# mahdi-slh/DeformContact

Hardware: AMD Instinct MI355X
Metric: M edges/sec fwd+bwd, everyday-deform batch=32 per GPU (encoder hot path) (higher is better)
Workload: dtype f32 (hops, storage, accumulate); wide dense blocks fp16x2-split operands (3 fp16 MFMA products, fp32 accumulate), narrow ones bf16x3-split (6 products); 1 GPU; everyday-deform synthetic, B=32 sample pairs per GPU: soft 32x(1024 v, 6132 e) + rigid 32x(762 v, 4560 e); TAGConv encoder 2 layers/branch, hidden 256, K=3 (configs[1]); edges_per_gpu_step=342144, global_batch=32, settle_steps=150, hipgraph=True, two_stream_branches=True, merged_branches=False, segmented_adjacency_build=True, parallelism=dp1

## Files before the change

### deformcontact_amd/_lib.py

```python
from __future__ import annotations

import ctypes
import os
from ctypes import POINTER, c_char_p, c_float, c_int, c_int32, c_int64, c_void_p

_HERE = os.path.dirname(os.path.abspath(__file__))
SO_PATH = os.path.join(_HERE, "libdeformcontact_hip.so")

_lib = None

_vp = c_void_p
_SIGNATURES = {
    "dc_version": (c_int, []),
    "dc_last_error": (c_char_p, []),
    "dc_stream_capture_id": (c_int64, [_vp]),
    "dc_csr_workspace_bytes": (c_int64, [c_int64, c_int64]),
    "dc_csr_build": (c_int, [_vp, c_int64, c_int64, c_int, c_int, _vp, _vp, _vp, _vp, _vp, _vp,
                             _vp, c_int64, _vp]),
    "dc_graph_workspace_bytes": (c_int64, [c_int64, c_int64]),
    "dc_graph_build": (c_int, [_vp, c_int64, c_int64, c_int, _vp, _vp, _vp, _vp, _vp, _vp, _vp, _vp,
                               _vp, _vp, c_int64, _vp]),
    "dc_graph_build_parts": (c_int, [POINTER(_vp), POINTER(c_int64), POINTER(c_int64), POINTER(c_int64), c_int,
                                     c_int64, c_int, _vp, _vp, _vp, _vp, _vp, _vp, _vp, _vp, _vp, _vp, c_int64,
                                     _vp]),
# ... 12 lines not shown
                                             _vp]),
    "dc_attn_flash_fwd": (c_int, [_vp, c_int64, _vp, _vp, _vp, _vp, _vp, c_int64, c_int64, c_int64, c_int64, _vp,
                                  c_int64, _vp, _vp]),
    "dc_hop_chain_max_nodes": (c_int64, []),
    "dc_hop_chain_lds_request": (c_int64, []),
    "dc_hop_chain_f32": (c_int, [_vp, _vp, _vp, _vp, c_int64, POINTER(c_int64), c_int, _vp, c_int64, c_int64, c_int64,
                                 c_int, c_int, c_int, _vp, c_int, _vp]),
    "dc_spmm_f32_bias_act": (c_int, [_vp, _vp, _vp, _vp, c_int64, _vp, c_int, _vp, c_int64, c_int64, c_int64, _vp]),
    "dc_colsum_workspace_bytes": (c_int64, [c_int64, c_int64, c_int]),
    "dc_mask_colsum_f32": (c_int, [_vp, c_int64, _vp, c_int64, _vp, c_int64, c_int64, c_int64, _vp, c_int64, _vp, c_int,
                                   _vp]),
    "dc_gat_alpha_fwd": (c_int, [_vp, c_int64, _vp, _vp, _vp, _vp, c_int64, c_int64, _vp]),
    "dc_gat_alpha_bwd": (c_int, [_vp, c_int64, _vp, _vp, _vp, _vp, _vp, c_int64, c_int64, c_int64, _vp, c_int64, _vp, _vp,
                                 c_int, _vp]),
    "dc_spmm_f32_pack": (c_int, [_vp, _vp, _vp, _vp, c_int64, _vp, c_int64, c_int64, c_int64, c_int64, c_int64, _vp]),
    "dc_spmm_f32_window": (c_int, [_vp, _vp, _vp, _vp, c_int64, _vp, c_int64, _vp, c_int64, c_int64,
                                   c_int64, c_int64, _vp]),
    "dc_spmm_f32_rowmax_window": (c_int, [_vp, _vp, _vp, _vp, c_int64, _vp, c_int64, _vp, c_int64, c_int64,
                                          c_int64, _vp, c_int, c_int64, _vp]),
    "dc_tag_grouped_weight_prep": (c_int, [POINTER(_vp), c_int, c_int, c_int64, c_int64, POINTER(_vp),
                                           POINTER(_vp), POINTER(_vp), POINTER(_vp), _vp]),
    "dc_tag_grouped_fwd_h2p": (c_int, [_vp, c_int64, c_int, POINTER(c_int64), POINTER(c_int64), c_int64,
                                       POINTER(_vp), POINTER(_vp), c_int, _vp, c_int64, c_int64, c_int64, _vp,
                                       POINTER(_vp), _vp]),
    "dc_tag_grouped_mask_grad": (c_int, [POINTER(_vp), POINTER(c_int64), c_int, POINTER(c_int64),
                                         POINTER(c_int64), c_int64, _vp, c_int64, _vp, c_int64, c_int64, _vp,
                                         _vp, _vp]),
    "dc_tag_grouped_bwd_dw_workspace_bytes": (c_int64, [POINTER(c_int64), c_int, c_int64, c_int64, c_int]),
    "dc_tag_grouped_bwd_dw_h2": (c_int, [_vp, c_int64, POINTER(_vp), POINTER(c_int64), c_int, c_int,
                                         POINTER(c_int64), POINTER(c_int64), c_int64, POINTER(_vp),
# ... 63 lines not shown
    "dc_tag_linear_fwd_h2p": (c_int, [_vp, c_int64, _vp, _vp, c_int, _vp, c_int64, c_int64, c_int64, c_int64,
                                      _vp, _vp, _vp, c_int64, _vp]),
    "dc_tag_linear_fwd_h2p_exp": (c_int, [_vp, c_int64, _vp, _vp, c_int64, c_int64, c_int64, c_int64, _vp, _vp, _vp,
                                          c_int64, _vp]),
    "dc_tag_weight_prep": (c_int, [POINTER(_vp), c_int, c_int64, c_int64, _vp, _vp, _vp, _vp, _vp]),
    "dc_tag_weight_prep_zero": (c_int, [POINTER(_vp), c_int, c_int64, c_int64, _vp, _vp, _vp, _vp, _vp, c_int64, _vp]),
    "dc_rowabsmax_f32": (c_int, [_vp, c_int64, c_int64, c_int64, _vp, _vp]),
    "dc_tag_weight_rowmax": (c_int, [POINTER(_vp), c_int, c_int64, c_int64, _vp, _vp]),
    "dc_spmm_f32_rowmax": (c_int, [_vp, _vp, _vp, _vp, c_int64, _vp, c_int64, _vp, c_int64, c_int64,
                                   c_int64, _vp, c_int, _vp]),
    "dc_tag_pack_input": (c_int, [_vp, c_int64, _vp, c_int64, c_int64, c_int64, c_int64, c_int64, _vp]),
    "dc_tag_pack_weights": (c_int, [POINTER(_vp), c_int, _vp, c_int64, c_int64, c_int64, _vp]),
    "dc_tag_linear_fwd_narrow_ok": (c_int, [c_int64, c_int, c_int64, c_int64]),
    "dc_tag_linear_fwd_narrow": (c_int, [_vp, c_int64, POINTER(_vp), c_int, c_int64, _vp, c_int, _vp, c_int64, c_int64,
                                         c_int64, c_int64, _vp]),
    "dc_attn_softmax_rows": (c_int, [_vp, c_int64, c_int64, c_int64, c_int64, _vp, _vp]),
    "dc_attn_exp_rows": (c_int, [_vp, c_int64, c_int64, c_int64, c_int64, _vp, _vp]),
    "dc_attn_ds_rows": (c_int, [_vp, _vp, c_int64, c_int64, c_int64, _vp, _vp, _vp]),
    "dc_adam_flat": (c_int, [_vp, _vp, _vp, _vp, c_int64, _vp, c_float, c_float, c_float, c_float,
                             c_int, _vp]),
    "dc_compose_perm": (c_int, [_vp, _vp, _vp, _vp, c_int64, _vp]),
    "dc_gat_edge_softmax_fwd": (c_int, [_vp, _vp, _vp, _vp, c_float, _vp, c_int64, _vp]),
    "dc_gat_edge_softmax_bwd": (c_int, [_vp, _vp, _vp, _vp, c_float, _vp, _vp, _vp, _vp, c_int64,
                                        _vp]),
    "dc_sddmm_f32": (c_int, [_vp, _vp, _vp, c_int64, _vp, c_int64, _vp, c_int64, c_int64, _vp]),
    "dc_segment_sum_f32": (c_int, [_vp, _vp, _vp, _vp, c_int64, _vp]),
    "dc_gather_f32": (c_int, [_vp, _vp, _vp, _vp, c_int64, _vp]),
    "dc_gat_alpha_heads_fwd": (c_int, [_vp, c_int64, _vp, _vp, _vp, _vp, c_int64, c_int64, c_int64, _vp]),
    "dc_gat_edge_softmax_heads_fwd": (c_int, [_vp, _vp, _vp, _vp, c_float, _vp, c_int64, c_int64, _vp]),
    "dc_spmm_f32_heads_bias_act": (c_int, [_vp, _vp, _vp, _vp, c_int64, _vp, c_int, c_int, _vp, c_int64, c_int64,
# ... 134 lines not shown
```

### deformcontact_amd/csrc/dc_dense_narrow.hip

```cpp
#include "dc_dense.h"

#ifndef DC_NARROW_ABL
#define DC_NARROW_ABL 0
#endif

namespace dc {

struct NarrowParams {
    const float *x;
    int64_t ld;
    const float *w[kMaxSeg];
    int nseg, fi;
    const float *bias;
    float *out;
    int64_t ldo, N;
    int relu, ntiles;
};

constexpr int kNarrowFo = 256;


template <int KS, int MB>
__global__ void __launch_bounds__(256)
k_fwd_narrow(NarrowParams p) {
    constexpr int TR = 32 * MB;
    constexpr int SROWA = KS * 96 + 16;
    constexpr int PPR = 4 * KS;
    constexpr int TP = TR * PPR, NV = (TP + 255) / 256;
    constexpr int KP = 16 * KS;
    constexpr int kOffStage = ((TR * SROWA + 1023) / 1024) * 1024;
    constexpr int kLdsTiles = kOffStage + TR * 1024, kLdsW = kNarrowFo * (KP + 4) * 4;
    __shared__ __attribute__((aligned(1024))) char lds[kLdsTiles > kLdsW ? kLdsTiles : kLdsW];
    char *const sA = lds;
    float *const so = reinterpret_cast<float *>(lds + kOffStage);
    const int wid = __builtin_amdgcn_readfirstlane((int)(threadIdx.x >> 6)), lane = threadIdx.x & 63;
    const int c = lane & 31, h = lane >> 5;

    f32x4 xv[NV];
    auto load_tile = [&](int t) {
        const int64_t row0 = (int64_t)t * TR;
#pragma unroll
        for (int j = 0; j < NV; ++j) {
            const int q = (int)threadIdx.x + 256 * j;
            if (TP % 256 != 0 && q >= TP) continue;
            const int r = q / PPR, c4 = q - r * PPR;
            int64_t row = row0 + r;
            row = row < p.N ? row : p.N - 1;
            if (DC_NARROW_ABL & 8) xv[j] = f32x4{(float)row, 1.f, 2.f, 3.f};
            else xv[j] = *reinterpret_cast<const f32x4 *>(p.x + row * p.ld + 4 * c4);
        }
    };
    int t = blockIdx.x;
    if (t < p.ntiles) load_tile(t);

    constexpr int WROW = KP + 4;
    {
        float *wi = reinterpret_cast<float *>(lds);
        const int width = p.nseg * p.fi, per4 = kNarrowFo * p.fi / 4;
        constexpr int MAXQ = 8;
        f32x4 wv[kMaxSeg][MAXQ];
#pragma unroll
        for (int s = 0; s < kMaxSeg; ++s)
#pragma unroll
            for (int j = 0; j < MAXQ; ++j) {
                const int q = (int)threadIdx.x + 256 * j;
                if (!(DC_NARROW_ABL & 2) && s < p.nseg && q < per4) wv[s][j] = *reinterpret_cast<const f32x4 *>(p.w[s] + 4 * q);
            }
#pragma unroll
        for (int s = 0; s < kMaxSeg; ++s)
#pragma unroll
// ... 3 lines not shown
                    int o = (4 * q) / p.fi, f = 4 * q - o * p.fi;
#pragma unroll
                    for (int i = 0; i < 4; ++i) {
                        wi[o * WROW + s * p.fi + f] = wv[s][j][i];
                        if (++f == p.fi) f = 0, ++o;
                    }
                }
            }
        const int padw = KP - width;
        for (int e = threadIdx.x; e < kNarrowFo * padw; e += 256) {
            const int o = e / padw, f = e - o * padw;
            wi[o * WROW + width + f] = 0.f;
        }
    }
    __syncthreads();
    bf16x8 fb[2][KS][3];
#pragma unroll
    for (int nb = 0; nb < 2; ++nb) {
        const float *wr = reinterpret_cast<const float *>(lds) + (64 * wid + 32 * nb + c) * WROW + 8 * h;
#pragma unroll
        for (int ks = 0; ks < KS; ++ks) {
            const f32x4 v0 = *reinterpret_cast<const f32x4 *>(wr + 16 * ks);
            const f32x4 v1 = *reinterpret_cast<const f32x4 *>(wr + 16 * ks + 4);
#pragma unroll
            for (int j = 0; j < 8; ++j) {
                __bf16 hi, mid, lo;
                split1(j < 4 ? v0[j] : v1[j - 4], hi, mid, lo);
                fb[nb][ks][0][j] = hi, fb[nb][ks][1][j] = mid, fb[nb][ks][2][j] = lo;
            }
        }
    }
    __syncthreads();
    float bcol[2];
#pragma unroll
    for (int nb = 0; nb < 2; ++nb) bcol[nb] = p.bias ? p.bias[64 * wid + 32 * nb + c] : 0.f;
    const bool relu = p.relu != 0;

    auto store_tile = [&]() {
#pragma unroll
        for (int j = 0; j < NV; ++j) {
            const int q = (int)threadIdx.x + 256 * j;
            if (TP % 256 != 0 && q >= TP) continue;
            const int r = q / PPR, c4 = q - r * PPR;
            bf16x4 hi, mid, lo;
#pragma unroll
            for (int i = 0; i < 4; ++i) {
                __bf16 a, b, d;
// ... 8 lines not shown
    };

    auto store_rows = [&](int64_t row0) {
#pragma unroll 4
        for (int r = wid; r < TR; r += 4) {
            const int64_t row = row0 + r;
            const f32x4 v = *reinterpret_cast<const f32x4 *>(so + r * 256 + 4 * lane);
            if (row < p.N && (!(DC_NARROW_ABL & 4) || v[0] == 12345.678f)) *reinterpret_cast<f32x4 *>(p.out + row * p.ldo + 4 * lane) = v;
        }
    };
    int64_t prev_row0 = -1;
    for (; t < p.ntiles; t += gridDim.x) {
        const int64_t row0 = (int64_t)t * TR;
        if (!(DC_NARROW_ABL & 8)) store_tile();
        if (prev_row0 >= 0) store_rows(prev_row0);
        if (t + (int)gridDim.x < p.ntiles) load_tile(t + gridDim.x);
        lds_barrier();
        f32x16 acc[MB][2];
#pragma unroll
        for (int mb = 0; mb < MB; ++mb)
#pragma unroll
            for (int nb = 0; nb < 2; ++nb)
#pragma unroll
                for (int i = 0; i < 16; ++i) acc[mb][nb][i] = 0.f;
        constexpr int HI = 0, MID = 1, LO = 2;
        constexpr int pa6[6] = {LO, HI, MID, MID, HI, HI}, pb6[6] = {HI, LO, MID, HI, MID, HI};
#pragma unroll
        for (int ks = 0; ks < KS; ++ks) {
            bf16x8 fa[MB][3];
#pragma unroll
            for (int mb = 0; mb < MB; ++mb)
#pragma unroll
                for (int pl = 0; pl < 3; ++pl)
                    fa[mb][pl] = *reinterpret_cast<const bf16x8 *>(sA + (mb * 32 + c) * SROWA + ks * 96 + pl * 32 + h * 16);
#pragma unroll
            for (int tt = 0; tt < 6; ++tt)
#pragma unroll
                for (int mb = 0; mb < MB; ++mb)
#pragma unroll
                    for (int nb = 0; nb < 2; ++nb)
                        if (!(DC_NARROW_ABL & 1))
                            acc[mb][nb] = __builtin_amdgcn_mfma_f32_32x32x16_bf16(fa[mb][pa6[tt]], fb[nb][ks][pb6[tt]], acc[mb][nb], 0, 0, 0);
                        else
                            acc[mb][nb][tt] += (float)fa[mb][pa6[tt]][0] * (float)fb[nb][ks][pb6[tt]][0];
        }
#pragma unroll
        for (int mb = 0; mb < MB; ++mb)
#pragma unroll
            for (int nb = 0; nb < 2; ++nb)
#pragma unroll
                for (int r = 0; r < 16; ++r) {
                    float v = acc[mb][nb][r] + bcol[nb];
                    if (relu) v = fmaxf(v, 0.f);
                    if (!(DC_NARROW_ABL & 16) || r == 0)
                        so[(mb * 32 + (r & 3) + 8 * (r >> 2) + 4 * h) * 256 + 64 * wid + 32 * nb + c] = v;
                }
        lds_barrier();
        prev_row0 = row0;
    }
    if (prev_row0 >= 0) store_rows(prev_row0);
}

template <int KS>
static void narrow_launch(const NarrowParams &p0, hipStream_t hs) {
    NarrowParams p = p0;
    p.ntiles = (int)((p.N + 31) / 32);
    const unsigned grid = (unsigned)(p.ntiles < 256 ? p.ntiles : 256);
    DC_LAUNCH((k_fwd_narrow<KS, 1>), dim3(grid), dim3(256), 0, hs, p);
}

}

using namespace dc;

extern "C" int dc_tag_linear_fwd_narrow_ok(int64_t fi, int nseg, int64_t wpad, int64_t Fo) {
// ... 5 lines not shown
                                        const float *bias, int relu, float *out, int64_t ldo, int64_t N, int64_t wpad,
                                        int64_t Fo, dc_stream_t stream) {
    DC_REQUIRE(dc_tag_linear_fwd_narrow_ok(fi, nseg, wpad, Fo),
               "dc_tag_linear_fwd_narrow: needs Fo = 256, a padded reduction of 96 / 112 / 128 >= nseg * fi (got Fo=%lld wpad=%lld "
               "nseg=%d fi=%lld)", (long long)Fo, (long long)wpad, nseg, (long long)fi);
    DC_REQUIRE(N >= 0, "dc_tag_linear_fwd_narrow: negative N");
    if (N == 0) return DC_OK;
    DC_REQUIRE(slab && ws && out && ld >= wpad && ldo >= Fo, "dc_tag_linear_fwd_narrow: null pointer / short leading dimension");
    DC_REQUIRE(ld % 4 == 0 && ldo % 4 == 0 && ((uintptr_t)slab & 15) == 0 && ((uintptr_t)out & 15) == 0,
               "dc_tag_linear_fwd_narrow: rows of the slab and of the output must be 16-byte aligned");
    DC_REQUIRE(N < ((int64_t)1 << 31) - 64, "dc_tag_linear_fwd_narrow: too many rows");
    NarrowParams p{};
    p.x = slab, p.ld = ld, p.nseg = nseg, p.fi = (int)fi, p.bias = bias, p.out = out, p.ldo = ldo, p.N = N, p.relu = relu;
    for (int s = 0; s < nseg; ++s) {
        DC_REQUIRE(ws[s], "dc_tag_linear_fwd_narrow: null weight segment %d", s);
        p.w[s] = ws[s];
    }
    hipStream_t hs = (hipStream_t)stream;
    switch (wpad) {
    case 96: narrow_launch<6>(p, hs); break;
    case 112: narrow_launch<7>(p, hs); break;
    default: narrow_launch<8>(p, hs); break;
    }
    return check_launch("dc_tag_linear_fwd_narrow");
}
```

### deformcontact_amd/csrc/dc_spmm.hip

```cpp
#include <stdlib.h>

#include "dc_common.h"

#pragma clang fp contract(off)

namespace dc {

template <int VEC> struct Vec;
template <> struct Vec<1> { using T = float; };
template <> struct Vec<4> { using T = float4; };

__device__ __forceinline__ float vzero(float) { return 0.0f; }
__device__ __forceinline__ float4 vzero(float4) { return make_float4(0.f, 0.f, 0.f, 0.f); }

__device__ __forceinline__ void vaxpy(float &acc, float w, float v) {
    const float m = w * v;
    acc = acc + m;
}
__device__ __forceinline__ void vaxpy(float4 &acc, float w, const float4 &v) {
    const float mx = w * v.x, my = w * v.y, mz = w * v.z, mw = w * v.w;
    acc.x = acc.x + mx;
    acc.y = acc.y + my;
    acc.z = acc.z + mz;
    acc.w = acc.w + mw;
// ... 102 lines not shown
        ww[3] = row_share_f<3>(my_w), ww[4] = row_share_f<4>(my_w), ww[5] = row_share_f<5>(my_w);
        ww[6] = row_share_f<6>(my_w), ww[7] = row_share_f<7>(my_w);
    } else {
        const bool mine = sub < 8 && p + sub < end;
        const int my_s = mine ? other[p + sub] : 0;
        const float my_w = mine ? (w ? w[p + sub] : 1.0f) : 0.0f;
#pragma unroll
        for (int j = 0; j < 8; ++j) {
            s[j] = __shfl(my_s, j, L);
            ww[j] = __shfl(my_w, j, L);
        }
    }
}

template <int VEC, int L, int U>
__global__ void __launch_bounds__(256)
k_spmm_sub(const int32_t *__restrict__ ptr, const int32_t *__restrict__ other,
           const float *__restrict__ w, const float *__restrict__ x, int64_t ldx,
           const float *addend, int64_t ldadd, float *y, int64_t ldy,
           int64_t N, int F, int src_off, float *self_dst = nullptr, int pad_beg = 0, int pad_end = 0) {
    using V = typename Vec<VEC>::T;
    constexpr int kRows = 256 / L;
    const unsigned lb = xcd_remap(blockIdx.x, gridDim.x);
    const int64_t row = (int64_t)lb * kRows + threadIdx.x / L;
    if (row >= N) return;
    const int sub = threadIdx.x % L;
    const int beg = ptr[row], end = ptr[row + 1];
    if (self_dst) {
        for (int c = sub; c < F; c += L) self_dst[row * ldy + c] = x[row * ldx + c];
        for (int c = pad_beg + sub; c < pad_end; c += L) self_dst[row * ldy + c] = 0.f;
    }

    for (int c0 = 0; c0 < F; c0 += L * VEC) {
        const int c = c0 + sub * VEC;
        const bool act = c < F;
        V acc = (addend && act) ? *reinterpret_cast<const V *>(addend + row * ldadd + c) : vzero(V{});
        for (int p = beg; p < end; p += U) {
            int s[U];
// ... 8 lines not shown
                    s[j] = ok ? other[p + j] : 0;
                    ww[j] = ok ? (w ? w[p + j] : 1.0f) : 0.0f;
                }
            }
#pragma unroll
            for (int j = 0; j < U; ++j) {
                const bool ok = act && p + j < end;
                v[j] = ok ? *reinterpret_cast<const V *>(x + (int64_t)(s[j] - src_off) * ldx + c) : vzero(V{});
            }
#pragma unroll
            for (int j = 0; j < U; ++j)
                if (p + j < end) vaxpy(acc, ww[j], v[j]);
        }
        if (act) *reinterpret_cast<V *>(y + row * ldy + c) = acc;
    }
}

template <int VEC, int L, int U>
static void launch_sub(const int32_t *ptr, const int32_t *other, const float *w, const float *x,
                       int64_t ldx, const float *addend, int64_t ldadd, float *y, int64_t ldy,
                       int64_t N, int F, int src_off, hipStream_t stream, float *self_dst = nullptr,
                       int pad_beg = 0, int pad_end = 0) {
    constexpr int kRows = 256 / L;
    const unsigned grid = (unsigned)((N + kRows - 1) / kRows);
    DC_LAUNCH((k_spmm_sub<VEC, L, U>), dim3(grid), dim3(256), 0, stream, ptr, other, w, x,
                       ldx, addend, ldadd, y, ldy, N, F, src_off, self_dst, pad_beg, pad_end);
}

static inline bool aligned16(const void *p) { return ((uintptr_t)p & 15) == 0; }

// ... 331 lines not shown
    if (N == 0) return DC_OK;
    DC_REQUIRE(ptr && x && slab && (other || true), "dc_spmm_f32_pack: null pointer");
    DC_REQUIRE(N < (int64_t)INT32_MAX / 8 && ldx >= F && width >= 2 * F && wpad >= width && lds >= wpad,
               "dc_spmm_f32_pack: needs ldx >= F, width >= 2 F (block 1 exists), wpad >= width, lds >= wpad");
    DC_REQUIRE((const void *)x != (const void *)slab, "dc_spmm_f32_pack: the slab must not alias x");
    float *y = slab + F;
    if (F > 16)
        launch_sub<1, 32, 8>(ptr, other, w, x, ldx, nullptr, 0, y, lds, N, (int)F, 0, stream, slab, (int)width, (int)wpad);
    else if (F > 8)
        launch_sub<1, 16, 8>(ptr, other, w, x, ldx, nullptr, 0, y, lds, N, (int)F, 0, stream, slab, (int)width, (int)wpad);
    else
        launch_sub<1, 8, 8>(ptr, other, w, x, ldx, nullptr, 0, y, lds, N, (int)F, 0, stream, slab, (int)width, (int)wpad);
    return check_launch("dc_spmm_f32_pack");
}

extern "C" int dc_spmm_f32_window(const int32_t *ptr, const int32_t *other, const float *w,
                                  const float *x, int64_t ldx, const float *addend, int64_t ldadd,
                                  float *y, int64_t ldy, int64_t N, int64_t F, int64_t row_offset,
                                  dc_stream_t stream) {
    DC_REQUIRE(row_offset >= 0 && row_offset < (int64_t)INT32_MAX, "dc_spmm_f32_window: bad row_offset");
    return spmm_f32_impl(ptr, other, w, x, ldx, addend, ldadd, y, ldy, N, F, (int)row_offset, stream);
}

extern "C" int dc_spmm_bf16(const int32_t *ptr, const int32_t *other, const float *w,
                            const uint16_t *x, int64_t ldx, const void *addend, int64_t ldadd,
                            void *y, int64_t ldy, int64_t N, int64_t F, int y_is_f32,
                            dc_stream_t stream_) {
    hipStream_t stream = (hipStream_t)stream_;
    DC_REQUIRE(N >= 0 && F >= 0, "dc_spmm_bf16: negative size N=%lld F=%lld", (long long)N,
               (long long)F);
// ... 58 lines not shown
```

### deformcontact_amd/ops.py

```python
from __future__ import annotations

import ctypes
import math
import os
from typing import List, Optional

import torch

from . import _lib
from .deferred import resolve
from .graph import GraphIndex, SortedAdjacency, _require_cuda, capture_id, current_stream_ptr, graph_index


def _rowmajor(t: torch.Tensor, what: str, dtypes=(torch.float32,)) -> int:
    if t.dim() != 2 or t.dtype not in dtypes:
        raise ValueError(f"{what}: expected a 2-D tensor of {dtypes}, got {tuple(t.shape)} {t.dtype}")
    if t.size(1) > 1 and t.stride(1) != 1:
        raise ValueError(f"{what}: innermost dimension must be contiguous")
    return t.stride(0) if t.size(0) > 1 else max(t.stride(0), t.size(1))


def _vp_array(ptrs):
    return (ctypes.c_void_p * len(ptrs))(*ptrs)

# ... 113 lines not shown
    return g if (ok and g.stride(1) == 1) else g.contiguous()


MAX_SEG = 4

DIRECT_PARAM_GRAD = True


DENSE_SPLIT_BF16 = os.environ.get("DC_DENSE_SPLIT", "1") != "0"

DENSE_PRODUCTS = 6


NARROW_FWD = os.environ.get("DC_NARROW_FWD", "1") != "0"

DENSE_F16X2 = os.environ.get("DC_DENSE_F16X2", "1") != "0"


HOP_CHAIN = os.environ.get("DC_HOP_CHAIN", "1") != "0"
_CHAIN_MAX_NODES = None


def hop_chain_eligible(g, adj: SortedAdjacency, slab: torch.Tensor, f: int, k: int) -> bool:
    global _CHAIN_MAX_NODES
    seg = getattr(g, "_layout", None)
    if not HOP_CHAIN or seg is None or k < 1 or f % 32 != 0 or adj.row_offset:
        return False
    if _CHAIN_MAX_NODES is None:
        _CHAIN_MAX_NODES = int(_lib.lib().dc_hop_chain_max_nodes())
    return (0 < g._seg_max_nodes <= _CHAIN_MAX_NODES and slab.dtype == torch.float32 and slab.dim() == 2
# ... 62 lines not shown
        return slab, rowmax
    return None


def _hop_cache_put(g, key, x, slab, rowmax, dev):
    cache = g.__dict__.setdefault("_hop_cache", {})
    if key not in cache:
        while len(cache) >= _HOP_CACHE_ENTRIES:
            cache.pop(next(iter(cache)))
    cache[key] = (slab, rowmax, capture_id(dev), x, x._version)


FUSED_PACK = os.environ.get("DC_FUSED_PACK", "1") != "0"


def _build_input_slab(g: GraphIndex, x: torch.Tensor, k: int, want_rowmax: bool, into=None):
    n, fi = x.shape
    concat, width, wpad = tag_slab_geometry(fi, k)
    dev = x.device
    slab = into[0] if into is not None else _alloc_slab(n, wpad, dev)
    xin = x if (x.dim() == 2 and x.stride(1) == 1) else x.contiguous()
    adj = g.fwd if (g is not None and k >= 1) else None
    if (FUSED_PACK and adj is not None and not want_rowmax and fi <= 32 and not adj.row_offset and g.normalize
            and adj.ptr.numel() == n + 1):
        _lib.check(_lib.lib().dc_spmm_f32_pack(adj.ptr.data_ptr(), adj.other.data_ptr(), adj.w.data_ptr(),
                                               xin.data_ptr(), xin.stride(0), slab.data_ptr(), slab.stride(0), n, fi,
                                               width, wpad, current_stream_ptr(dev)), "dc_spmm_f32_pack")
        for j in range(1, k):
            hop(adj, slab[:, j * fi:(j + 1) * fi], out=slab[:, (j + 1) * fi:(j + 2) * fi], weighted=True)
        return slab, None
    _lib.check(_lib.lib().dc_tag_pack_input(xin.data_ptr(), xin.stride(0), slab.data_ptr(), slab.stride(0), n,
                                            fi, width, wpad, current_stream_ptr(dev)),
               "dc_tag_pack_input")
    rowmax = None
    if want_rowmax:
        rowmax = into[1] if into is not None else torch.empty(n, dtype=torch.float32, device=dev)
    chained_hops(g, slab, fi, k, backward=False, rowmax=rowmax)
    return slab, rowmax


def _tag_uses_h2(fi: int, k: int, fo: Optional[int] = None) -> bool:
    concat, _, wpad = tag_slab_geometry(fi, k)
# ... 103 lines not shown
        return "fp32"
    if _tag_uses_h2(fi, k, None if six else fo):
        return "h2"
    if not tag_slab_geometry(fi, k)[0]:
        return "split"
    return "narrow" if (NARROW_FWD and DENSE_PRODUCTS == 6 and narrow_ok) else "concat"


def _dense_operands(slab: torch.Tensor, fi: int, k: int, concat: bool):
    ld = slab.stride(0)
    if concat:
        return [slab], [ld], slab.size(1), 1
    return [slab[:, j * fi:(j + 1) * fi] for j in range(k + 1)], [ld] * (k + 1), fi, k + 1


def _tag_slab(g, x: torch.Tensor, weights, h2: bool, need_x: bool):
    n, fi = x.shape
    k = len(weights) - 1
    dev = x.device
    wpad = tag_slab_geometry(fi, k)[2]
    slab = _as_slab_block0(x, n, fi, wpad)
    if slab is None and k == 0 and wpad == fi and x.is_contiguous() and x.data_ptr() % 16 == 0:
        slab = x
    rowmax = prepped = None
    if slab is None:
        key = None
        if HOP_CACHE and g is not None and k >= 1 and not need_x:
            key = _hop_cache_key(x, k, wpad, h2)
            hit = _hop_cache_get(g, key, x, dev)
            if hit is not None:
                slab, rowmax = hit
        if slab is None:
            slab, rowmax = _build_input_slab(g, x, k, h2)
            if key is not None:
                _hop_cache_put(g, key, x, slab, rowmax, dev)
    else:
        rowmax = torch.empty(n, dtype=torch.float32, device=dev) if h2 else None
        zeroed = False
        if h2 and g is not None and hop_chain_eligible(g, g.fwd, slab, fi, k):
            fo = weights[0].size(0)
            prepped = _h2_weight_prep(_lib.lib(), [w.contiguous() for w in weights], k, fo, fi,
                                      need_x and fo % 16 == 0, dev, current_stream_ptr(dev), zero=rowmax)
            zeroed = True
        chained_hops(g, slab, fi, k, backward=False, rowmax=rowmax, rowmax_zeroed=zeroed)
    if h2 and k == 0:
        rowmax = rowabsmax(slab)
    return slab, rowmax, prepped

# ... 143 lines not shown
            raise NotImplementedError(f"TAGConv K={k} > {MAX_SEG - 1} is not supported by the fused dense block")
        dev = x.device
        L = _lib.lib()
        st = current_stream_ptr(dev)
        six = next_geom is SIX_PRODUCTS
        if six:
            next_geom = None
        ctx.empty = n == 0
        if ctx.empty:
            ctx.fi, ctx.has_bias = fi, bias is not None
            ctx.save_for_backward(*weights)
            return _tag_out_buffer(next_geom, n, fo, dev)
        concat, width, wpad = tag_slab_geometry(fi, k)
        path = _dense_path(fi, k, fo, six, concat and bool(L.dc_tag_linear_fwd_narrow_ok(fi, k + 1, wpad, fo)))
        need_x = ctx.needs_input_grad[1]
        slab, rowmax, prepped = _tag_slab(g, x, weights, path == "h2", need_x)
        ws = [w.contiguous() for w in weights]
        if concat and path != "narrow":
            ws = [_pack_weights(ws, fo, fi, wpad, st)]
        out = _tag_out_buffer(next_geom, n, fo, dev)
        ldo = out.stride(0)
        b = bias.contiguous() if bias is not None else None
        wt = wt_rowmax = None
        if path == "h2":
            if prepped is None:
                prepped = _h2_weight_prep(L, ws, k, fo, fi, need_x and fo % 16 == 0, dev, st)
            wmax, wimg, wt, wt_rowmax = prepped
            rc = L.dc_tag_linear_fwd_h2p(slab.data_ptr(), slab.stride(0), wimg.data_ptr(), _ptr(b), int(relu),
                                         out.data_ptr(), ldo, n, width, fo, rowmax.data_ptr(), wmax.data_ptr(),
                                         None, 0, st)
        elif path == "narrow":
            rc = L.dc_tag_linear_fwd_narrow(slab.data_ptr(), slab.stride(0), _ptr_array(ws), k + 1, fi, _ptr(b),
                                            int(relu), out.data_ptr(), ldo, n, wpad, fo, st)
        else:
            xs, ldxs, fi_eff, nseg = _dense_operands(slab, fi, k, concat)
            args = (_ptr_array(xs), _i64_array(ldxs), _ptr_array(ws), nseg, _ptr(b), int(relu), out.data_ptr(), ldo,
                    n, fi_eff, fo)
            rc = L.dc_tag_linear_fwd(*args, st) if path == "fp32" else L.dc_tag_linear_fwd_split(*args, DENSE_PRODUCTS, st)
        _lib.check(rc, "dc_tag_linear_fwd")
        ctx.g, ctx.k, ctx.fi, ctx.fo, ctx.has_bias, ctx.relu, ctx.concat, ctx.path = \
            g, k, fi, fo, bias is not None, relu, concat, path
        ctx.params, ctx.bias_param = weights, bias
        ctx.save_for_backward(slab, out if relu else None, rowmax, wt, wt_rowmax, *ws)
        return out

# ... 2024 lines not shown
```

### include/deformcontact.h

```cpp
#ifndef DEFORMCONTACT_H
#define DEFORMCONTACT_H

#include <stdint.h>

#ifdef __cplusplus
extern "C" {
#endif

#define DC_OK 0
#define DC_EINVAL (-1)
#define DC_ELAUNCH (-2)
#define DC_EWORKSPACE (-3)

typedef void *dc_stream_t;

#define DC_MAX_PARTS 4
#define DC_MAX_GROUPS 4
#define DC_GROUP_ALIGN 256

int dc_version(void);
const char *dc_last_error(void);
int64_t dc_stream_capture_id(dc_stream_t stream);

int64_t dc_csr_workspace_bytes(int64_t E, int64_t N);
// ... 55 lines not shown

#define DC_NEIGHBORS_ND_CHUNK 32
int dc_neighbors_nd_fill(const float *x, int64_t ldx, int64_t nx, const int64_t *batch_x, const float *y, int64_t ldy,
                         int64_t ny, const int64_t *batch_y, int64_t f, int cap, int exclude_self, int32_t *nbr,
                         int32_t *counts, dc_stream_t stream);

int dc_hash_i64(const int64_t *v, int64_t n, uint64_t *out, dc_stream_t stream);

int dc_spmm_f32(const int32_t *ptr, const int32_t *other, const float *w, const float *x,
                int64_t ldx, const float *addend, int64_t ldadd, float *y, int64_t ldy,
                int64_t N, int64_t F, dc_stream_t stream);

int dc_spmm_f32_pack(const int32_t *ptr, const int32_t *other, const float *w, const float *x, int64_t ldx,
                     float *slab, int64_t lds, int64_t N, int64_t F, int64_t width, int64_t wpad,
                     dc_stream_t stream);

int dc_spmm_f32_window(const int32_t *ptr, const int32_t *other, const float *w, const float *x,
                       int64_t ldx, const float *addend, int64_t ldadd, float *y, int64_t ldy,
                       int64_t N, int64_t F, int64_t row_offset, dc_stream_t stream);
int dc_spmm_f32_rowmax_window(const int32_t *ptr, const int32_t *other, const float *w, const float *x,
                              int64_t ldx, const float *addend, int64_t ldadd, float *y, int64_t ldy,
                              int64_t N, int64_t F, float *rowmax, int mode, int64_t row_offset,
                              dc_stream_t stream);

int dc_spmm_bf16(const int32_t *ptr, const int32_t *other, const float *w, const uint16_t *x,
                 int64_t ldx, const void *addend, int64_t ldadd, void *y, int64_t ldy, int64_t N,
                 int64_t F, int y_is_f32, dc_stream_t stream);

int dc_spmm_f32_rowmax(const int32_t *ptr, const int32_t *other, const float *w, const float *x,
                       int64_t ldx, const float *addend, int64_t ldadd, float *y, int64_t ldy,
// ... 31 lines not shown
                      int nseg, const float *bias, int relu, float *out, int64_t ldo,
                      int64_t N, int64_t Fi, int64_t Fo, dc_stream_t stream);

int dc_tag_linear_bwd_dx(const float *g, int64_t ldg, const float *out_for_mask, int64_t ldo,
                         const float *const *ws, int nseg, float *const *gxs,
                         const int64_t *ldgxs, int64_t N, int64_t Fi, int64_t Fo,
                         dc_stream_t stream);

int dc_tag_linear_fwd_split(const float *const *xs, const int64_t *ldxs, const float *const *ws,
                            int nseg, const float *bias, int relu, float *out, int64_t ldo,
                            int64_t N, int64_t Fi, int64_t Fo, int products, dc_stream_t stream);
int dc_tag_linear_fwd_narrow_ok(int64_t fi, int nseg, int64_t wpad, int64_t Fo);
int dc_tag_linear_fwd_narrow(const float *slab, int64_t ld, const float *const *ws, int nseg, int64_t fi,
                             const float *bias, int relu, float *out, int64_t ldo, int64_t N, int64_t wpad,
                             int64_t Fo, dc_stream_t stream);
int64_t dc_tag_linear_bwd_dx_split_workspace_bytes(int64_t Fi, int64_t Fo, int nseg);
int dc_tag_linear_bwd_dx_split(const float *g, int64_t ldg, const float *out_for_mask,
                               int64_t ldo, const float *const *ws, int nseg, float *const *gxs,
                               const int64_t *ldgxs, void *workspace, int64_t workspace_bytes,
                               int64_t N, int64_t Fi, int64_t Fo, int products, dc_stream_t stream);

int64_t dc_tag_linear_bwd_dw_workspace_bytes(int64_t N, int64_t Fi, int64_t Fo, int nseg);
int dc_tag_linear_bwd_dw(const float *g, int64_t ldg, const float *out_for_mask, int64_t ldo,
                         const float *const *xs, const int64_t *ldxs, int nseg,
                         float *const *gws, int ngw, int64_t gw_cols, float *gbias,
                         int accumulate, void *partials, int64_t partials_bytes, int64_t N,
                         int64_t Fi, int64_t Fo, dc_stream_t stream);
int dc_tag_linear_bwd_dw_split(const float *g, int64_t ldg, const float *out_for_mask,
                               int64_t ldo, const float *const *xs, const int64_t *ldxs, int nseg,
                               float *const *gws, int ngw, int64_t gw_cols, float *gbias,
// ... 304 lines not shown
```

Measured before the change: 545.9 M edges/s.

## Prebuild narrow bf16x3 weight image inside pack kernel and read it in narrow fwd

Instead of having every block of the narrow TAG forward kernel load fp32 weights into LDS and split them into bf16 hi/mid/lo fragments, a precomputed fragment image is built once per forward. That build is fused as extra blocks into the SpMM pack kernel, so it costs no extra launch. The narrow kernel then reads per-lane fragments straight from global memory, which drops the weight-staging LDS and one barrier. It also adds launch_bounds occupancy variants (2 waves/CU for KS 6/7) and an option to defer the next-tile prefetch for KS>6. The risks are extra register pressure and the global image reads.

```diff
diff --git a/deformcontact_amd/_lib.py b/deformcontact_amd/_lib.py
--- a/deformcontact_amd/_lib.py
+++ b/deformcontact_amd/_lib.py
@@ -50,6 +50,8 @@
     "dc_gat_alpha_bwd": (c_int, [_vp, c_int64, _vp, _vp, _vp, _vp, _vp, c_int64, c_int64, c_int64, _vp, c_int64, _vp, _vp,
                                  c_int, _vp]),
     "dc_spmm_f32_pack": (c_int, [_vp, _vp, _vp, _vp, c_int64, _vp, c_int64, c_int64, c_int64, c_int64, c_int64, _vp]),
+    "dc_spmm_f32_pack_wprep": (c_int, [_vp, _vp, _vp, _vp, c_int64, _vp, c_int64, c_int64, c_int64, c_int64, c_int64,
+                                       POINTER(_vp), c_int, _vp, _vp]),
     "dc_spmm_f32_window": (c_int, [_vp, _vp, _vp, _vp, c_int64, _vp, c_int64, _vp, c_int64, c_int64,
                                    c_int64, c_int64, _vp]),
     "dc_spmm_f32_rowmax_window": (c_int, [_vp, _vp, _vp, _vp, c_int64, _vp, c_int64, _vp, c_int64, c_int64,
@@ -143,6 +145,8 @@
     "dc_tag_linear_fwd_narrow_ok": (c_int, [c_int64, c_int, c_int64, c_int64]),
     "dc_tag_linear_fwd_narrow": (c_int, [_vp, c_int64, POINTER(_vp), c_int, c_int64, _vp, c_int, _vp, c_int64, c_int64,
                                          c_int64, c_int64, _vp]),
+    "dc_tag_narrow_wimage": (c_int, [POINTER(_vp), c_int, c_int64, c_int64, _vp, _vp]),
+    "dc_tag_linear_fwd_narrow_img": (c_int, [_vp, c_int64, _vp, _vp, c_int, _vp, c_int64, c_int64, c_int64, c_int64, _vp]),
     "dc_attn_softmax_rows": (c_int, [_vp, c_int64, c_int64, c_int64, c_int64, _vp, _vp]),
     "dc_attn_exp_rows": (c_int, [_vp, c_int64, c_int64, c_int64, c_int64, _vp, _vp]),
     "dc_attn_ds_rows": (c_int, [_vp, _vp, c_int64, c_int64, c_int64, _vp, _vp, _vp]),
diff --git a/deformcontact_amd/csrc/dc_dense_narrow.hip b/deformcontact_amd/csrc/dc_dense_narrow.hip
--- a/deformcontact_amd/csrc/dc_dense_narrow.hip
+++ b/deformcontact_amd/csrc/dc_dense_narrow.hip
@@ -1,4 +1,5 @@
 #include "dc_dense.h"
+#include "dc_narrow_image.h"
 
 #ifndef DC_NARROW_ABL
 #define DC_NARROW_ABL 0
@@ -17,43 +18,13 @@
     int relu, ntiles;
 };
 
-constexpr int kNarrowFo = 256;
-
-
-template <int KS, int MB>
-__global__ void __launch_bounds__(256)
-k_fwd_narrow(NarrowParams p) {
-    constexpr int TR = 32 * MB;
-    constexpr int SROWA = KS * 96 + 16;
-    constexpr int PPR = 4 * KS;
-    constexpr int TP = TR * PPR, NV = (TP + 255) / 256;
+
+template <int KS>
+__device__ __forceinline__ void narrow_self_weights(const NarrowParams &p, char *lds, bf16x8 (&fb)[2][KS][3]) {
     constexpr int KP = 16 * KS;
-    constexpr int kOffStage = ((TR * SROWA + 1023) / 1024) * 1024;
-    constexpr int kLdsTiles = kOffStage + TR * 1024, kLdsW = kNarrowFo * (KP + 4) * 4;
-    __shared__ __attribute__((aligned(1024))) char lds[kLdsTiles > kLdsW ? kLdsTiles : kLdsW];
-    char *const sA = lds;
-    float *const so = reinterpret_cast<float *>(lds + kOffStage);
+    constexpr int WROW = KP + 4;
     const int wid = __builtin_amdgcn_readfirstlane((int)(threadIdx.x >> 6)), lane = threadIdx.x & 63;
     const int c = lane & 31, h = lane >> 5;
-
-    f32x4 xv[NV];
-    auto load_tile = [&](int t) {
-        const int64_t row0 = (int64_t)t * TR;
-#pragma unroll
-        for (int j = 0; j < NV; ++j) {
-            const int q = (int)threadIdx.x + 256 * j;
-            if (TP % 256 != 0 && q >= TP) continue;
-            const int r = q / PPR, c4 = q - r * PPR;
-            int64_t row = row0 + r;
-            row = row < p.N ? row : p.N - 1;
-            if (DC_NARROW_ABL & 8) xv[j] = f32x4{(float)row, 1.f, 2.f, 3.f};
-            else xv[j] = *reinterpret_cast<const f32x4 *>(p.x + row * p.ld + 4 * c4);
-        }
-    };
-    int t = blockIdx.x;
-    if (t < p.ntiles) load_tile(t);
-
-    constexpr int WROW = KP + 4;
     {
         float *wi = reinterpret_cast<float *>(lds);
         const int width = p.nseg * p.fi, per4 = kNarrowFo * p.fi / 4;
@@ -87,7 +58,6 @@
         }
     }
     __syncthreads();
-    bf16x8 fb[2][KS][3];
 #pragma unroll
     for (int nb = 0; nb < 2; ++nb) {
         const float *wr = reinterpret_cast<const float *>(lds) + (64 * wid + 32 * nb + c) * WROW + 8 * h;
@@ -104,6 +74,58 @@
         }
     }
     __syncthreads();
+}
+
+template <int KS, int MB, bool WIMG, bool LATE>
+__device__ __forceinline__ void narrow_block(const NarrowParams &p, const bf16x8 *__restrict__ img) {
+    constexpr int TR = 32 * MB;
+    constexpr int SROWA = KS * 96 + 16;
+    constexpr int PPR = 4 * KS;
+    constexpr int TP = TR * PPR, NV = (TP + 255) / 256;
+    constexpr int KP = 16 * KS;
+    constexpr int kOffStage = ((TR * SROWA + 1023) / 1024) * 1024;
+    constexpr int kLdsTiles = kOffStage + TR * 1024, kLdsW = kNarrowFo * (KP + 4) * 4;
+    __shared__ __attribute__((aligned(1024))) char lds[(WIMG || kLdsTiles > kLdsW) ? kLdsTiles : kLdsW];
+    char *const sA = lds;
+    float *const so = reinterpret_cast<float *>(lds + kOffStage);
+    const int wid = __builtin_amdgcn_readfirstlane((int)(threadIdx.x >> 6)), lane = threadIdx.x & 63;
+    const int c = lane & 31, h = lane >> 5;
+
+    f32x4 xv[NV];
+    auto load_tile = [&](int t) {
+        const int64_t row0 = (int64_t)t * TR;
+#pragma unroll
+        for (int j = 0; j < NV; ++j) {
+            const int q = (int)threadIdx.x + 256 * j;
+            if (TP % 256 != 0 && q >= TP) continue;
+            const int r = q / PPR, c4 = q - r * PPR;
+            int64_t row = row0 + r;
+            row = row < p.N ? row : p.N - 1;
+            if (DC_NARROW_ABL & 8) xv[j] = f32x4{(float)row, 1.f, 2.f, 3.f};
+            else xv[j] = *reinterpret_cast<const f32x4 *>(p.x + row * p.ld + 4 * c4);
+        }
+    };
+    int t = blockIdx.x;
+    if (t < p.ntiles) load_tile(t);
+
+    bf16x8 fb[2][KS][3];
+    if constexpr (WIMG) {
+#pragma unroll
+        for (int ks = 0; ks < KS; ++ks)
+#pragma unroll
+            for (int pl = 0; pl < 3; ++pl)
+#pragma unroll
+                for (int nb = 0; nb < 2; ++nb) {
+                    if (DC_NARROW_ABL & 2) {
+#pragma unroll
+                        for (int j = 0; j < 8; ++j) fb[nb][ks][pl][j] = (__bf16)(float)(lane + ks + pl + nb);
+                    } else {
+                        fb[nb][ks][pl] = img[((ks * 3 + pl) * 8 + 2 * wid + nb) * 64 + lane];
+                    }
+                }
+    } else {
+        narrow_self_weights<KS>(p, lds, fb);
+    }
     float bcol[2];
 #pragma unroll
     for (int nb = 0; nb < 2; ++nb) bcol[nb] = p.bias ? p.bias[64 * wid + 32 * nb + c] : 0.f;
@@ -142,7 +164,7 @@
         const int64_t row0 = (int64_t)t * TR;
         if (!(DC_NARROW_ABL & 8)) store_tile();
         if (prev_row0 >= 0) store_rows(prev_row0);
-        if (t + (int)gridDim.x < p.ntiles) load_tile(t + gridDim.x);
+        if (!LATE && t + (int)gridDim.x < p.ntiles) load_tile(t + gridDim.x);
         lds_barrier();
         f32x16 acc[MB][2];
 #pragma unroll
@@ -172,6 +194,7 @@
                         else
                             acc[mb][nb][tt] += (float)fa[mb][pa6[tt]][0] * (float)fb[nb][ks][pb6[tt]][0];
         }
+        if (LATE && t + (int)gridDim.x < p.ntiles) load_tile(t + gridDim.x);
 #pragma unroll
         for (int mb = 0; mb < MB; ++mb)
 #pragma unroll
@@ -187,6 +210,30 @@
         prev_row0 = row0;
     }
     if (prev_row0 >= 0) store_rows(prev_row0);
+}
+
+template <int KS, int MB>
+__global__ void __launch_bounds__(256) k_fwd_narrow(NarrowParams p) { narrow_block<KS, MB, false, false>(p, nullptr); }
+
+template <int KS, int WPC>
+__global__ void __launch_bounds__(256, WPC) k_fwd_narrow_img(NarrowParams p, const bf16x8 *__restrict__ img) {
+    narrow_block<KS, 1, true, (WPC == 2 && KS > 6)>(p, img);
+}
+
+__global__ void __launch_bounds__(256) k_narrow_wimage(NarrowImageParams q) { narrow_image_fill(q, (int)blockIdx.x); }
+
+static int narrow_wpc() {
+    static const int v = env_int("DC_NARROW_WPC", 2) == 1 ? 1 : 2;
+    return v;
+}
+
+template <int KS, int WPC>
+static void narrow_img_launch(const NarrowParams &p0, const void *img, hipStream_t hs) {
+    NarrowParams p = p0;
+    p.ntiles = (int)((p.N + 31) / 32);
+    const int cap = 256 * (WPC == 2 ? narrow_wpc() : 1);
+    const unsigned grid = (unsigned)(p.ntiles < cap ? p.ntiles : cap);
+    DC_LAUNCH((k_fwd_narrow_img<KS, WPC>), dim3(grid), dim3(256), 0, hs, p, static_cast<const bf16x8 *>(img));
 }
 
 template <int KS>
@@ -222,6 +269,7 @@
     p.x = slab, p.ld = ld, p.nseg = nseg, p.fi = (int)fi, p.bias = bias, p.out = out, p.ldo = ldo, p.N = N, p.relu = relu;
     for (int s = 0; s < nseg; ++s) {
         DC_REQUIRE(ws[s], "dc_tag_linear_fwd_narrow: null weight segment %d", s);
+        DC_REQUIRE(al16(ws[s]), "dc_tag_linear_fwd_narrow: weight segment %d is not 16-byte aligned", s);
         p.w[s] = ws[s];
     }
     hipStream_t hs = (hipStream_t)stream;
@@ -232,3 +280,37 @@
     }
     return check_launch("dc_tag_linear_fwd_narrow");
 }
+
+extern "C" int dc_tag_narrow_wimage(const float *const *ws, int nseg, int64_t fi, int64_t wpad, void *wimg,
+                                    dc_stream_t stream) {
+    DC_REQUIRE(narrow_image_args_ok(ws, nseg, fi, wpad, wimg),
+               "dc_tag_narrow_wimage: needs 1..%d 4-byte-aligned weight segments [256, fi <= 32], a padded reduction of 96 / "
+               "112 / 128 >= nseg * fi and a 16-byte-aligned image (got nseg=%d fi=%lld wpad=%lld)", kMaxSeg, nseg,
+               (long long)fi, (long long)wpad);
+    const NarrowImageParams q = narrow_image_params(ws, nseg, fi, wpad, wimg);
+    DC_LAUNCH(k_narrow_wimage, dim3((unsigned)narrow_image_blocks(q.ks)), dim3(256), 0, (hipStream_t)stream, q);
+    return check_launch("dc_tag_narrow_wimage");
+}
+
+extern "C" int dc_tag_linear_fwd_narrow_img(const float *slab, int64_t ld, const void *wimg, const float *bias, int relu,
+                                            float *out, int64_t ldo, int64_t N, int64_t wpad, int64_t Fo,
+                                            dc_stream_t stream) {
+    DC_REQUIRE(Fo == kNarrowFo && (wpad == 96 || wpad == 112 || wpad == 128),
+               "dc_tag_linear_fwd_narrow_img: needs Fo = 256 and a padded reduction of 96 / 112 / 128 (got Fo=%lld wpad=%lld)",
+               (long long)Fo, (long long)wpad);
+    DC_REQUIRE(N >= 0, "dc_tag_linear_fwd_narrow_img: negative N");
+    if (N == 0) return DC_OK;
+    DC_REQUIRE(slab && wimg && out && ld >= wpad && ldo >= Fo, "dc_tag_linear_fwd_narrow_img: null pointer / short leading dimension");
+    DC_REQUIRE(ld % 4 == 0 && ldo % 4 == 0 && al16(slab) && al16(out) && al16(wimg),
+               "dc_tag_linear_fwd_narrow_img: rows of the slab and of the output and the image must be 16-byte aligned");
+    DC_REQUIRE(N < ((int64_t)1 << 31) - 64, "dc_tag_linear_fwd_narrow_img: too many rows");
+    NarrowParams p{};
+    p.x = slab, p.ld = ld, p.bias = bias, p.out = out, p.ldo = ldo, p.N = N, p.relu = relu;
+    hipStream_t hs = (hipStream_t)stream;
+    switch (wpad) {
+    case 96: narrow_img_launch<6, 2>(p, wimg, hs); break;
+    case 112: narrow_img_launch<7, 2>(p, wimg, hs); break;
+    default: narrow_img_launch<8, 1>(p, wimg, hs); break;
+    }
+    return check_launch("dc_tag_linear_fwd_narrow_img");
+}
diff --git a/deformcontact_amd/csrc/dc_narrow_image.h b/deformcontact_amd/csrc/dc_narrow_image.h
--- /dev/null
+++ b/deformcontact_amd/csrc/dc_narrow_image.h
@@ -0,0 +1,66 @@
+#pragma once
+#include "dc_dense.h"
+
+namespace dc {
+
+constexpr int kNarrowFo = 256;
+constexpr int kNarrowImgStepBytes = 3 * 8 * 64 * 16;
+
+struct NarrowImageParams {
+    const float *w[kMaxSeg];
+    int nseg, fi, ks;
+    void *img;
+};
+
+__host__ __device__ constexpr int narrow_image_items(int ks) { return kNarrowFo * 2 * ks; }
+__host__ __device__ constexpr int narrow_image_blocks(int ks) { return narrow_image_items(ks) / 256; }
+
+__device__ __forceinline__ void narrow_image_fill(const NarrowImageParams &p, int blk) {
+    const int id = blk * 256 + (int)threadIdx.x;
+    const int per = 2 * p.ks;
+    const int o = id / per, kh = id - o * per;
+    if (o >= kNarrowFo) return;
+    const int width = p.nseg * p.fi;
+    float v[8];
+    int s = (8 * kh) / p.fi, f = 8 * kh - s * p.fi;
+#pragma unroll
+    for (int j = 0; j < 8; ++j) {
+        v[j] = 0.f;
+        if (8 * kh + j < width) {
+            const float *ws = p.w[0];
+#pragma unroll
+            for (int q = 1; q < kMaxSeg; ++q) ws = s == q ? p.w[q] : ws;
+            v[j] = ws[o * p.fi + f];
+        }
+        if (++f == p.fi) f = 0, ++s;
+    }
+    bf16x8 pl[3];
+#pragma unroll
+    for (int j = 0; j < 8; ++j) {
+        __bf16 hi, mid, lo;
+        split1(v[j], hi, mid, lo);
+        pl[0][j] = hi, pl[1][j] = mid, pl[2][j] = lo;
+    }
+    const int ks = kh >> 1, h = kh & 1, lane = (o & 31) + 32 * h;
+    char *dst = static_cast<char *>(p.img) + (size_t)ks * kNarrowImgStepBytes + ((o >> 5) * 64 + lane) * 16;
+#pragma unroll
+    for (int q = 0; q < 3; ++q) *reinterpret_cast<bf16x8 *>(dst + q * (8 * 64 * 16)) = pl[q];
+}
+
+inline bool narrow_image_args_ok(const float *const *ws, int nseg, int64_t fi, int64_t wpad, const void *img) {
+    if (!ws || !img || nseg < 1 || nseg > kMaxSeg || fi < 1 || fi > 32 || nseg * fi > wpad) return false;
+    if (wpad != 96 && wpad != 112 && wpad != 128) return false;
+    if ((uintptr_t)img & 15) return false;
+    for (int s = 0; s < nseg; ++s)
+        if (!ws[s] || ((uintptr_t)ws[s] & 3)) return false;
+    return true;
+}
+
+inline NarrowImageParams narrow_image_params(const float *const *ws, int nseg, int64_t fi, int64_t wpad, void *img) {
+    NarrowImageParams q{};
+    for (int s = 0; s < nseg; ++s) q.w[s] = ws[s];
+    q.nseg = nseg, q.fi = (int)fi, q.ks = (int)(wpad / 16), q.img = img;
+    return q;
+}
+
+}
diff --git a/deformcontact_amd/csrc/dc_spmm.hip b/deformcontact_amd/csrc/dc_spmm.hip
--- a/deformcontact_amd/csrc/dc_spmm.hip
+++ b/deformcontact_amd/csrc/dc_spmm.hip
@@ -1,6 +1,7 @@
 #include <stdlib.h>
 
 #include "dc_common.h"
+#include "dc_narrow_image.h"
 
 #pragma clang fp contract(off)
 
@@ -140,14 +141,13 @@
 }
 
 template <int VEC, int L, int U>
-__global__ void __launch_bounds__(256)
-k_spmm_sub(const int32_t *__restrict__ ptr, const int32_t *__restrict__ other,
-           const float *__restrict__ w, const float *__restrict__ x, int64_t ldx,
-           const float *addend, int64_t ldadd, float *y, int64_t ldy,
-           int64_t N, int F, int src_off, float *self_dst = nullptr, int pad_beg = 0, int pad_end = 0) {
+__device__ __forceinline__ void
+spmm_sub_rows(unsigned lb, const int32_t *__restrict__ ptr, const int32_t *__restrict__ other,
+              const float *__restrict__ w, const float *__restrict__ x, int64_t ldx,
+              const float *addend, int64_t ldadd, float *y, int64_t ldy,
+              int64_t N, int F, int src_off, float *self_dst, int pad_beg, int pad_end) {
     using V = typename Vec<VEC>::T;
     constexpr int kRows = 256 / L;
-    const unsigned lb = xcd_remap(blockIdx.x, gridDim.x);
     const int64_t row = (int64_t)lb * kRows + threadIdx.x / L;
     if (row >= N) return;
     const int sub = threadIdx.x % L;
@@ -186,6 +186,30 @@
         }
         if (act) *reinterpret_cast<V *>(y + row * ldy + c) = acc;
     }
+}
+
+template <int VEC, int L, int U>
+__global__ void __launch_bounds__(256)
+k_spmm_sub(const int32_t *__restrict__ ptr, const int32_t *__restrict__ other,
+           const float *__restrict__ w, const float *__restrict__ x, int64_t ldx,
+           const float *addend, int64_t ldadd, float *y, int64_t ldy,
+           int64_t N, int F, int src_off, float *self_dst = nullptr, int pad_beg = 0, int pad_end = 0) {
+    spmm_sub_rows<VEC, L, U>(xcd_remap(blockIdx.x, gridDim.x), ptr, other, w, x, ldx, addend, ldadd, y, ldy, N, F, src_off,
+                             self_dst, pad_beg, pad_end);
+}
+
+template <int L, int U>
+__global__ void __launch_bounds__(256)
+k_spmm_sub_wimg(const int32_t *__restrict__ ptr, const int32_t *__restrict__ other,
+                const float *__restrict__ w, const float *__restrict__ x, int64_t ldx, float *y, int64_t ldy,
+                int64_t N, int F, float *self_dst, int pad_beg, int pad_end, NarrowImageParams img) {
+    const unsigned nimg = (unsigned)narrow_image_blocks(img.ks);
+    if (blockIdx.x < nimg) {
+        narrow_image_fill(img, (int)blockIdx.x);
+        return;
+    }
+    spmm_sub_rows<1, L, U>(xcd_remap(blockIdx.x - nimg, gridDim.x - nimg), ptr, other, w, x, ldx, nullptr, 0, y, ldy, N, F, 0,
+                           self_dst, pad_beg, pad_end);
 }
 
 template <int VEC, int L, int U>
@@ -547,6 +571,40 @@
     return check_launch("dc_spmm_f32_pack");
 }
 
+template <int L>
+static void launch_pack_wimg(const int32_t *ptr, const int32_t *other, const float *w, const float *x, int64_t ldx,
+                             float *slab, int64_t lds, int64_t N, int F, int width, int wpad,
+                             const NarrowImageParams &img, hipStream_t stream) {
+    constexpr int kRows = 256 / L;
+    const unsigned grid = (unsigned)((N + kRows - 1) / kRows) + (unsigned)narrow_image_blocks(img.ks);
+    DC_LAUNCH((k_spmm_sub_wimg<L, 8>), dim3(grid), dim3(256), 0, stream, ptr, other, w, x, ldx, slab + F, lds, N, F, slab,
+              width, wpad, img);
+}
+
+extern "C" int dc_spmm_f32_pack_wprep(const int32_t *ptr, const int32_t *other, const float *w, const float *x,
+                                      int64_t ldx, float *slab, int64_t lds, int64_t N, int64_t F, int64_t width,
+                                      int64_t wpad, const float *const *ws, int nseg, void *wimg, dc_stream_t stream_) {
+    hipStream_t stream = (hipStream_t)stream_;
+    DC_REQUIRE(N >= 1 && F >= 1 && F <= 32, "dc_spmm_f32_pack_wprep: at least one row of 1..32 floats (got N=%lld F=%lld)",
+               (long long)N, (long long)F);
+    DC_REQUIRE(ptr && x && slab, "dc_spmm_f32_pack_wprep: null pointer");
+    DC_REQUIRE(N < (int64_t)INT32_MAX / 8 && ldx >= F && width >= 2 * F && wpad >= width && lds >= wpad,
+               "dc_spmm_f32_pack_wprep: needs ldx >= F, width >= 2 F (block 1 exists), wpad >= width, lds >= wpad");
+    DC_REQUIRE((const void *)x != (const void *)slab, "dc_spmm_f32_pack_wprep: the slab must not alias x");
+    DC_REQUIRE(width == (int64_t)nseg * F && narrow_image_args_ok(ws, nseg, F, wpad, wimg),
+               "dc_spmm_f32_pack_wprep: needs 1..%d 4-byte-aligned weight segments with nseg * F = width, a padded width of "
+               "96 / 112 / 128 and a 16-byte-aligned image (got nseg=%d F=%lld width=%lld wpad=%lld)", kMaxSeg, nseg,
+               (long long)F, (long long)width, (long long)wpad);
+    const NarrowImageParams img = narrow_image_params(ws, nseg, F, wpad, wimg);
+    if (F > 16)
+        launch_pack_wimg<32>(ptr, other, w, x, ldx, slab, lds, N, (int)F, (int)width, (int)wpad, img, stream);
+    else if (F > 8)
+        launch_pack_wimg<16>(ptr, other, w, x, ldx, slab, lds, N, (int)F, (int)width, (int)wpad, img, stream);
+    else
+        launch_pack_wimg<8>(ptr, other, w, x, ldx, slab, lds, N, (int)F, (int)width, (int)wpad, img, stream);
+    return check_launch("dc_spmm_f32_pack_wprep");
+}
+
 extern "C" int dc_spmm_f32_window(const int32_t *ptr, const int32_t *other, const float *w,
                                   const float *x, int64_t ldx, const float *addend, int64_t ldadd,
                                   float *y, int64_t ldy, int64_t N, int64_t F, int64_t row_offset,
diff --git a/deformcontact_amd/ops.py b/deformcontact_amd/ops.py
--- a/deformcontact_amd/ops.py
+++ b/deformcontact_amd/ops.py
@@ -151,6 +151,25 @@
 
 NARROW_FWD = os.environ.get("DC_NARROW_FWD", "1") != "0"
 
+NARROW_PREP = os.environ.get("DC_NARROW_PREP", "1") != "0"
+
+
+class _NarrowImage:
+
+    STEP_BYTES = 3 * 8 * 64 * 16
+
+    def __init__(self, ws, wpad: int, dev):
+        self.ws, self.wpad, self.filled = ws, wpad, False
+        self.buf = torch.empty(wpad // 16 * self.STEP_BYTES, dtype=torch.uint8, device=dev)
+
+    def ensure(self, st) -> int:
+        if not self.filled:
+            fi = self.ws[0].size(1)
+            _lib.check(_lib.lib().dc_tag_narrow_wimage(_ptr_array(self.ws), len(self.ws), fi, self.wpad,
+                                                       self.buf.data_ptr(), st), "dc_tag_narrow_wimage")
+            self.filled = True
+        return self.buf.data_ptr()
+
 DENSE_F16X2 = os.environ.get("DC_DENSE_F16X2", "1") != "0"
 
 
@@ -243,7 +262,7 @@
 FUSED_PACK = os.environ.get("DC_FUSED_PACK", "1") != "0"
 
 
-def _build_input_slab(g: GraphIndex, x: torch.Tensor, k: int, want_rowmax: bool, into=None):
+def _build_input_slab(g: GraphIndex, x: torch.Tensor, k: int, want_rowmax: bool, into=None, nimg=None):
     n, fi = x.shape
     concat, width, wpad = tag_slab_geometry(fi, k)
     dev = x.device
@@ -252,9 +271,14 @@
     adj = g.fwd if (g is not None and k >= 1) else None
     if (FUSED_PACK and adj is not None and not want_rowmax and fi <= 32 and not adj.row_offset and g.normalize
             and adj.ptr.numel() == n + 1):
-        _lib.check(_lib.lib().dc_spmm_f32_pack(adj.ptr.data_ptr(), adj.other.data_ptr(), adj.w.data_ptr(),
-                                               xin.data_ptr(), xin.stride(0), slab.data_ptr(), slab.stride(0), n, fi,
-                                               width, wpad, current_stream_ptr(dev)), "dc_spmm_f32_pack")
+        args = (adj.ptr.data_ptr(), adj.other.data_ptr(), adj.w.data_ptr(), xin.data_ptr(), xin.stride(0),
+                slab.data_ptr(), slab.stride(0), n, fi, width, wpad)
+        if nimg is not None and not nimg.filled and len(nimg.ws) == k + 1:
+            _lib.check(_lib.lib().dc_spmm_f32_pack_wprep(*args, _ptr_array(nimg.ws), k + 1, nimg.buf.data_ptr(),
+                                                         current_stream_ptr(dev)), "dc_spmm_f32_pack_wprep")
+            nimg.filled = True
+        else:
+            _lib.check(_lib.lib().dc_spmm_f32_pack(*args, current_stream_ptr(dev)), "dc_spmm_f32_pack")
         for j in range(1, k):
             hop(adj, slab[:, j * fi:(j + 1) * fi], out=slab[:, (j + 1) * fi:(j + 2) * fi], weighted=True)
         return slab, None
@@ -388,7 +412,7 @@
     return [slab[:, j * fi:(j + 1) * fi] for j in range(k + 1)], [ld] * (k + 1), fi, k + 1
 
 
-def _tag_slab(g, x: torch.Tensor, weights, h2: bool, need_x: bool):
+def _tag_slab(g, x: torch.Tensor, weights, h2: bool, need_x: bool, nimg=None):
     n, fi = x.shape
     k = len(weights) - 1
     dev = x.device
@@ -405,7 +429,7 @@
             if hit is not None:
                 slab, rowmax = hit
         if slab is None:
-            slab, rowmax = _build_input_slab(g, x, k, h2)
+            slab, rowmax = _build_input_slab(g, x, k, h2, nimg=nimg)
             if key is not None:
                 _hop_cache_put(g, key, x, slab, rowmax, dev)
     else:
@@ -579,8 +603,9 @@
         concat, width, wpad = tag_slab_geometry(fi, k)
         path = _dense_path(fi, k, fo, six, concat and bool(L.dc_tag_linear_fwd_narrow_ok(fi, k + 1, wpad, fo)))
         need_x = ctx.needs_input_grad[1]
-        slab, rowmax, prepped = _tag_slab(g, x, weights, path == "h2", need_x)
         ws = [w.contiguous() for w in weights]
+        nimg = _NarrowImage(ws, wpad, dev) if (path == "narrow" and NARROW_PREP) else None
+        slab, rowmax, prepped = _tag_slab(g, x, weights, path == "h2", need_x, nimg)
         if concat and path != "narrow":
             ws = [_pack_weights(ws, fo, fi, wpad, st)]
         out = _tag_out_buffer(next_geom, n, fo, dev)
@@ -594,6 +619,9 @@
             rc = L.dc_tag_linear_fwd_h2p(slab.data_ptr(), slab.stride(0), wimg.data_ptr(), _ptr(b), int(relu),
                                          out.data_ptr(), ldo, n, width, fo, rowmax.data_ptr(), wmax.data_ptr(),
                                          None, 0, st)
+        elif path == "narrow" and nimg is not None:
+            rc = L.dc_tag_linear_fwd_narrow_img(slab.data_ptr(), slab.stride(0), nimg.ensure(st), _ptr(b), int(relu),
+                                                out.data_ptr(), ldo, n, wpad, fo, st)
         elif path == "narrow":
             rc = L.dc_tag_linear_fwd_narrow(slab.data_ptr(), slab.stride(0), _ptr_array(ws), k + 1, fi, _ptr(b),
                                             int(relu), out.data_ptr(), ldo, n, wpad, fo, st)
diff --git a/include/deformcontact.h b/include/deformcontact.h
--- a/include/deformcontact.h
+++ b/include/deformcontact.h
@@ -93,6 +93,9 @@
 int dc_spmm_f32_pack(const int32_t *ptr, const int32_t *other, const float *w, const float *x, int64_t ldx,
                      float *slab, int64_t lds, int64_t N, int64_t F, int64_t width, int64_t wpad,
                      dc_stream_t stream);
+int dc_spmm_f32_pack_wprep(const int32_t *ptr, const int32_t *other, const float *w, const float *x, int64_t ldx,
+                           float *slab, int64_t lds, int64_t N, int64_t F, int64_t width, int64_t wpad,
+                           const float *const *ws, int nseg, void *wimg, dc_stream_t stream);
 
 int dc_spmm_f32_window(const int32_t *ptr, const int32_t *other, const float *w, const float *x,
                        int64_t ldx, const float *addend, int64_t ldadd, float *y, int64_t ldy,
@@ -154,6 +157,9 @@
 int dc_tag_linear_fwd_narrow(const float *slab, int64_t ld, const float *const *ws, int nseg, int64_t fi,
                              const float *bias, int relu, float *out, int64_t ldo, int64_t N, int64_t wpad,
                              int64_t Fo, dc_stream_t stream);
+int dc_tag_narrow_wimage(const float *const *ws, int nseg, int64_t fi, int64_t wpad, void *wimg, dc_stream_t stream);
+int dc_tag_linear_fwd_narrow_img(const float *slab, int64_t ld, const void *wimg, const float *bias, int relu,
+                                 float *out, int64_t ldo, int64_t N, int64_t wpad, int64_t Fo, dc_stream_t stream);
 int64_t dc_tag_linear_bwd_dx_split_workspace_bytes(int64_t Fi, int64_t Fo, int nseg);
 int dc_tag_linear_bwd_dx_split(const float *g, int64_t ldg, const float *out_for_mask,
                                int64_t ldo, const float *const *ws, int nseg, float *const *gxs,
```

Measured after the change: 554.9 M edges/s (median of 6 runs). +1.7%, better.
